# yeyupiaoling/MASR

Measured on AMD Instinct MI355X. Metric: audio-seconds/sec (RTF^-1), conformer_streaming_fbank b32x10s, PCM->fbank->encoder->ctc_greedy->text, higher is better.
Workload: dtype f32; 1 GPU; configs[1]: conformer.yml streaming fbank, batch=32 synthetic 16 kHz 10 s utterances per GPU, ctc_greedy, random-init weights V=4233; global_batch=32, parallelism=dp1, world_size_observed=1, backend=none

## Files before the change

include/masr_hip.h:

```cpp
#ifndef MASR_HIP_H
#define MASR_HIP_H
#include <stdint.h>
#ifdef __cplusplus
extern "C" {
#endif

typedef struct masr_engine masr_engine;

typedef struct masr_config {
    int32_t model_kind;
    int32_t d_model;
    int32_t heads;
    int32_t d_ff;
    int32_t num_blocks;
    int32_t cnn_kernel;
    int32_t n_mels;
    int32_t vocab_size;
    int32_t causal;
    int32_t max_pos;
    int32_t device_id;
    int32_t reserved[5];
} masr_config;

const char* masr_last_error(void);
// ... 121 lines not shown

int masr_stream_open(masr_engine* e, int32_t max_frames_out, int32_t* stream_id);
int masr_stream_reset(masr_engine* e, int32_t stream_id);
int masr_stream_close(masr_engine* e, int32_t stream_id);
int masr_stream_set_history(masr_engine* e, int32_t stream_id, int32_t required_cache_size);
int masr_stream_offset(masr_engine* e, int32_t stream_id, int32_t* offset);
int masr_stream_cache_len(masr_engine* e, int32_t stream_id, int32_t* cache_len);
int masr_stream_room(masr_engine* e, int32_t stream_id, int32_t* frames_left);

int masr_stage_rows(void* dst, int64_t row_bytes, const void* const* src, const int32_t* n_samples, int32_t B, int32_t sample_bytes,
                    int32_t threads);

int masr_resample_f32(const float* x, int64_t n_orig, double ratio, const double* win, const double* dwin, int64_t nwin,
                      int32_t num_table, float* y, int64_t n_out);
int masr_resample_rows(masr_engine* e, const void* src_dev, int32_t sample_format, int64_t src_stride, const int32_t* rows_host,
                       const int32_t* rows_dev, int32_t R, double ratio, const double* table_dev, int64_t nwin, int32_t num_table,
                       float* dst_dev, int32_t dst_rows, int64_t dst_stride, void* stream);
int masr_encode_chunk(masr_engine* e, const int32_t* stream_ids, int32_t n, const float* feats_dev, int32_t Tc,
                      float* probs_dev, int32_t* argmax_dev, float* maxprob_dev, void* stream);
int masr_stream_export_cache(masr_engine* e, int32_t stream_id, float* att_dev, float* cnn_dev, void* stream);

int masr_op_layernorm(masr_engine* e, const float* x_dev, const float* w_dev, const float* b_dev, float* y_dev,
                      int32_t M, float eps, void* stream);
int masr_op_gemm(masr_engine* e, const float* a_dev, const float* w_dev, const float* bias_dev, const float* res_dev,
                 float* c_dev, int32_t M, int32_t N, int32_t K, int32_t act, float alpha, void* stream);

#define MASR_SIDE_STREAMS 5
int masr_side_stream(masr_engine* e, int32_t kind, void** stream_out);

#define MASR_LANES 2
int masr_select_lane(masr_engine* e, int32_t lane);

int masr_debug_set(masr_engine* e, int32_t key, int32_t value);

int masr_profile_select(masr_engine* e, int32_t kind);
int masr_profile_read(masr_engine* e, double* total_ms, int64_t* launches, double* flops, int32_t reset);

int masr_mfma_order_probe(const float* a_dev, const float* b_dev, float* c32_dev, float* c16_dev, int32_t k, const int32_t* perm,
                          void* stream);

#ifdef __cplusplus
}
#endif
#endif
```

masr_amd/_lib.py:

```python
import ctypes as C
import os

from .build import LIB_PATH

_lib = None


class MasrConfig(C.Structure):
    _fields_ = [('model_kind', C.c_int32), ('d_model', C.c_int32), ('heads', C.c_int32), ('d_ff', C.c_int32),
                ('num_blocks', C.c_int32), ('cnn_kernel', C.c_int32), ('n_mels', C.c_int32),
                ('vocab_size', C.c_int32), ('causal', C.c_int32), ('max_pos', C.c_int32), ('device_id', C.c_int32),
                ('reserved', C.c_int32 * 5)]


class MasrError(RuntimeError):
    pass


_P = C.c_void_p
_I = C.c_int32
_F = C.c_float

SIGNATURES = {
    'masr_last_error': [],
# ... 43 lines not shown
    'masr_vad_forward': [_P, _I, _P, _I, _I, _I, _P, _P, _P, _P],
    'masr_mean_square': [_P, _P, _I, _P, _I, _I, _P, _P],
    'masr_mfcc_batch': [_P, _P, _I, _P, _I, _I, _I, _F, _I, _P, _P, _P, _P],
    'masr_linear_batch': [_P, _P, _I, _P, _I, _I, _I, _F, _P, _P, _P, _P],
    'masr_transcribe_batch': [_P, _P, _P, _I, _I, _I, _F, _I, _P, _P, _P, _P],
    'masr_transcribe_rows': [_P, _P, _I, _P, _I, _I, _I, _F, _P, _I, _P, _P],
    'masr_pool_create': [_P, _I, _I, _I, _F, _I, C.POINTER(_P)],
    'masr_pool_destroy': [_P],
    'masr_pool_open': [_P, C.POINTER(_I)],
    'masr_pool_close': [_P, _I],
    'masr_pool_reset': [_P, _I],
    'masr_pool_step': [_P, _I, _P, _P, _P, _P, _P, _P, _P, C.POINTER(_I), C.POINTER(_P), C.POINTER(_P), C.POINTER(_P),
                       C.POINTER(_I), C.POINTER(_P), _P],
    'masr_pool_profile': [_P, C.POINTER(C.c_double), C.POINTER(C.c_int64), _I],
    'masr_encoder_frames': [_P, _I, C.POINTER(_I)],
    'masr_engine_info': [_P, C.POINTER(_I), C.POINTER(_I), C.POINTER(_I)],
    'masr_stream_open': [_P, _I, C.POINTER(_I)],
    'masr_stream_reset': [_P, _I],
    'masr_stream_close': [_P, _I],
    'masr_stream_offset': [_P, _I, C.POINTER(_I)],
    'masr_stream_cache_len': [_P, _I, C.POINTER(_I)],
    'masr_stream_room': [_P, _I, C.POINTER(_I)],
    'masr_resample_f32': [_P, C.c_int64, C.c_double, _P, _P, C.c_int64, _I, _P, C.c_int64],
    'masr_resample_rows': [_P, _P, _I, C.c_int64, _P, _P, _I, C.c_double, _P, C.c_int64, _I, _P, _I, C.c_int64, _P],
    'masr_stream_set_history': [_P, _I, _I],
    'masr_encode_chunk': [_P, C.POINTER(_I), _I, _P, _I, _P, _P, _P, _P],
    'masr_stream_export_cache': [_P, _I, _P, _P, _P],
    'masr_op_layernorm': [_P, _P, _P, _P, _P, _I, _F, _P],
    'masr_op_gemm': [_P, _P, _P, _P, _P, _P, _I, _I, _I, _I, _F, _P],
    'masr_side_stream': [_P, _I, C.POINTER(_P)],
    'masr_select_lane': [_P, _I],
    'masr_stage_rows': [_P, C.c_int64, _P, _P, _I, _I, _I],
    'masr_debug_set': [_P, _I, _I],
    'masr_mfma_order_probe': [_P, _P, _P, _P, _I, _P, _P],
    'masr_profile_select': [_P, _I],
    'masr_profile_read': [_P, C.POINTER(C.c_double), C.POINTER(C.c_int64), C.POINTER(C.c_double), _I],
}
_RESTYPE = {'masr_last_error': C.c_char_p, 'masr_destroy': None, 'masr_beam_destroy': None, 'masr_lm_destroy': None,
            'masr_lm_last_error': C.c_char_p, 'masr_vad_last_error': C.c_char_p, 'masr_vad_destroy': None, 'masr_pool_destroy': None}


GAIN_FN = C.CFUNCTYPE(C.c_int, C.POINTER(C.c_float), C.c_int32, C.c_float, C.POINTER(C.c_float), C.c_void_p)


def lib():
    global _lib
    if _lib is not None:
        return _lib
    import torch
    if not os.path.exists(LIB_PATH):
        raise MasrError(f'{LIB_PATH} not found: build it with `python -m masr_amd.build` '
                        f'(hipcc --offload-arch=gfx950). There is no CPU fallback.')
    h = C.CDLL(LIB_PATH)
    for name, args in SIGNATURES.items():
        fn = getattr(h, name)
        fn.argtypes = args
        fn.restype = _RESTYPE.get(name, C.c_int)
    _lib = h
    return h


def check(rc):
    if rc != 0:
        raise MasrError(lib().masr_last_error().decode('utf-8', 'replace'))
```

masr_amd/build.py:

```python
import os
import subprocess
from concurrent.futures import ThreadPoolExecutor

ROOT = os.path.dirname(os.path.abspath(__file__))
CSRC = os.path.join(ROOT, 'csrc')
LIB_DIR = os.path.join(ROOT, 'lib')
LIB_PATH = os.path.join(LIB_DIR, 'libmasr_hip.so')
SOURCES = ['gemm_f32.hip', 'ffn_reduce.hip', 'ffn_pc.hip', 'sqz_layer.hip', 'rowgemm.hip', 'rowgemm_small.hip', 'elementwise.hip',
           'attention.hip', 'lstm.hip', 'gru.hip', 'beam_gpu.hip', 'lm_scorer.cpp', 'fbank.hip', 'silero.hip', 'engine.hip', 'pool.hip',
           'beam_search.cpp', 'stage.cpp', 'resample.cpp', 'resample.hip']
EXPERIMENTS = os.environ.get('MASR_BUILD_EXPERIMENTS') == '1'
EXPERIMENT_SOURCES = ['gemm_bf16x3.hip', 'ffn_x3.hip', 'ffn_coop.hip', 'ffn_dual.hip']
if EXPERIMENTS:
    SOURCES = SOURCES + EXPERIMENT_SOURCES
HEADERS = [os.path.join(CSRC, 'common.h'), os.path.join(CSRC, 'lm_scorer.h'),
           os.path.join(os.path.dirname(ROOT), 'include', 'masr_hip.h')]
FLAGS = ['--offload-arch=gfx950', '-O3', '-std=c++17', '-fPIC', '-Wno-unused-value'] + (['-DMASR_EXPERIMENTS=1'] if EXPERIMENTS else [])
FILE_FLAGS = {'resample.hip': ['-ffp-contract=off', '-fno-gpu-flush-denormals-to-zero']}
STAMP = os.path.join(LIB_DIR, '.build_flavour')


def _hipcc():
    for c in (os.environ.get('HIPCC'), '/opt/rocm/bin/hipcc', 'hipcc'):
        if c and (os.path.isabs(c) and os.path.exists(c) or not os.path.isabs(c)):
            return c
    return 'hipcc'


def _sources():
    return [s for s in SOURCES if os.path.exists(os.path.join(CSRC, s))]


def _obj(src):
    stem, ext = os.path.splitext(src)
    if sum(os.path.splitext(s)[0] == stem for s in SOURCES) > 1:
        stem += '_' + ext[1:]
    return os.path.join(LIB_DIR, stem + '.o')


def _stale(src):
    obj = _obj(src)
# ... 60 lines not shown
```

masr_amd/csrc/common.h:

```cpp
#pragma once
#include <hip/hip_runtime.h>
#include <stdint.h>

#include "lm_scorer.h"

#ifndef MASR_EXPERIMENTS
#define MASR_EXPERIMENTS 0
#endif

typedef float f32x4 __attribute__((ext_vector_type(4)));
typedef float f32x16 __attribute__((ext_vector_type(16)));

namespace masr {

struct LdsAttr {
    size_t granted[32] = {};
};
void ensure_dynamic_lds(const void* fn, size_t bytes, LdsAttr& st);
void note_launch_error(const char* what, hipError_t e);

#ifdef __HIPCC__
struct SeqRow {
    int b, t;
};
__device__ __forceinline__ SeqRow seq_row(int b0, int t0, int T, int lr) {
    SeqRow r{b0, t0 + lr};
    while (r.t >= T) {
        r.t -= T;
        ++r.b;
    }
    return r;
}

__device__ __forceinline__ float wave_sum_dpp(float v) {
#define MASR_DPP_F(x, ctrl, rows) \
    __builtin_bit_cast(float, __builtin_amdgcn_update_dpp(0, __builtin_bit_cast(int, (x)), (ctrl), (rows), 0xf, false))
    v += MASR_DPP_F(v, 0x111, 0xf);
    v += MASR_DPP_F(v, 0x112, 0xf);
    v += MASR_DPP_F(v, 0x114, 0xf);
    v += MASR_DPP_F(v, 0x118, 0xf);
    v += MASR_DPP_F(v, 0x142, 0xa);
    v += MASR_DPP_F(v, 0x143, 0xc);
#undef MASR_DPP_F
    return __builtin_bit_cast(float, __builtin_amdgcn_readlane(__builtin_bit_cast(int, v), 63));
}
#endif


enum InputLayer { IL_CONV2D = 0, IL_CONV2D6 = 1, IL_CONV2D8 = 2 };
__host__ __device__ inline int sub_rate(int il) { return il == IL_CONV2D6 ? 6 : il == IL_CONV2D8 ? 8 : 4; }
__host__ __device__ inline int sub_min_frames(int il) { return il == IL_CONV2D6 ? 11 : il == IL_CONV2D8 ? 15 : 7; }
__host__ __device__ inline int sub_after_conv1(int il, int n1) {
    return il == IL_CONV2D6 ? (n1 - 2) / 3 : il == IL_CONV2D8 ? ((n1 - 1) / 2 - 1) / 2 : (n1 - 1) / 2;
}
__host__ __device__ inline int sub_frames(int il, int T) { return T < sub_min_frames(il) ? 0 : sub_after_conv1(il, (T - 1) / 2); }
__host__ __device__ inline int sub_bins(int il, int F) { return sub_after_conv1(il, (F - 1) / 2); }

enum GemmAct { ACT_NONE = 0, ACT_RELU = 1, ACT_SILU = 2 };
enum GemmAMode { A_PLAIN = 0, A_CONV2 = 1, A_CONV5 = 2 };
enum GemmEpi { EPI_STD = 0, EPI_GLU = 1, EPI_SPLITK = 2 };

struct GemmArgs {
    const float* A;
    const float* W;
    const float* bias;
    float* C;
    const float* R;
    const int* lens;
    int M, N, K;
    int lda, ldc, ldr;
    int act;
    float alpha;
    int mask_tp;
    int bias_after_alpha;
    int T1, F1, T2, F2, Cc;
    int nsplit, ksplit;
    int skip_rps, skip_div;
    const float* Wp;
// ... 123 lines not shown
    const float* lnb;
    const float* W;
    const float* bias;
    float* out;
    int N, ldo;
    const float* pre_lnw;
    const float* pre_lnb;
    long plane_stride;
    int seq_t, pad_t;
};
struct FfnHead {
    const float* glu;
    const float* dw_w;
    const float* dw_b;
    const float* lnw;
    const float* lnb;
    const float* gconst;
    const float* W;
    const float* bias;
    const int* lens;
    int seq_t, ktaps, mstride;
    float* xout;
};
int launch_ffn_fused(float* x, const float* lnw, const float* lnb, const float* w1, const float* b1, const float* w2,
                     const float* b2, int M, int dff, float eps, float scale, int affine_prologue, float* partial,
                     int nsplit, hipStream_t s, const FfnPostLn* post = nullptr, const FfnTail* tail = nullptr,
                     const FfnHead* head = nullptr, bool packed = false);
void launch_pack_ffn_pc(const float* w1, const float* w2, float* p1, float* p2, int dff, hipStream_t s);
void launch_pack_rows_pc(const float* w, float* p, int N, hipStream_t s, int n_src = -1);
int launch_ffn16(float* x, const float* lnw, const float* lnb, const float* w1, const float* b1, const float* w2, const float* b2, int M,
                 int dff, float eps, float scale, hipStream_t s, const FfnTail* tail, const FfnHead* head);
void launch_pack_ffn16(const float* w1, const float* w2, float* p1, float* p2, int dff, hipStream_t s);
void launch_pack_rows16(const float* w, float* p, int N, hipStream_t s, int n_src = -1);
struct SqzStageArgs {
    float* x;
    float* out;
    const float* att;
    const float* head_w;
    const float* head_b;
    const float *ln_a_w, *ln_a_b, *ln_b_w, *ln_b_b;
    const float *ffn_s, *ffn_b, *w1, *b1, *w2, *b2;
    const float *tail_w, *tail_b, *tail_s, *tail_sb;
    float* tail_out;
    float* glu_out;
    const float* glu;
    const float *dw_w, *dw_b, *bn_scale, *bn_shift, *gconst;
    const float* gpad;
    const int* lens;
    int M, dff, seq_t, mstride, ktaps, tail_n, glu_pad_l, glu_pad_tot;
    float eps;
    int skip_pad;
};
bool launch_sqz_stage(const SqzStageArgs& a, int stage, hipStream_t s);
#if MASR_EXPERIMENTS
int launch_ffn_dual(float* x, const float* lnw, const float* lnb, const float* p1, const float* b1, const float* p2,
                    const float* b2, int M, int dff, float eps, float scale, int affine_prologue, hipStream_t s,
                    const FfnTail* tail, const FfnHead* head);
void launch_pack_ffn_dual(const float* w1, const float* w2, float* p1, float* p2, int dff, hipStream_t s);
void launch_pack_rows_dual(const float* w, float* p, hipStream_t s);
#else
inline int launch_ffn_dual(float*, const float*, const float*, const float*, const float*, const float*, const float*, int, int, float,
                           float, int, hipStream_t, const FfnTail*, const FfnHead*) { return -1; }
inline void launch_pack_ffn_dual(const float*, const float*, float*, float*, int, hipStream_t) {}
inline void launch_pack_rows_dual(const float*, float*, hipStream_t) {}
#endif

// ... 129 lines not shown
```

masr_amd/csrc/engine.hip:

```cpp
#include <math.h>
#include <stdio.h>
#include <stdlib.h>
#include <string.h>

#include <map>
#include <mutex>
#include <string>
#include <vector>

#include "../../include/masr_hip.h"
#include "common.h"

using namespace masr;
namespace masr {
int lm_device_view(masr_lm* lm, LmView* out);
bool lm_word_based(const masr_lm* lm);
}
extern "C" const char* masr_lm_last_error(void);

static thread_local std::string g_err;
static int fail(const std::string& m) {
    g_err = m;
    return 1;
}
// ... 199 lines not shown
static int clear_sync(void* p, int value, size_t n) {
    HIPCHK(hipMemset(p, value, n));
    HIPCHK(hipStreamSynchronize(nullptr));
    return 0;
}

struct masr_engine : EngineWs {
    masr_config cfg;
    EngineWs parked[MASR_LANES];
    int lane = 0;
    hipEvent_t pack_ev = nullptr;
    void* pack_stream = nullptr;
    bool pack_pending = false;
    bool finalized = false;
    std::map<std::string, HostTensor> host;
    std::vector<void*> owned;
    float *cmvn_mean = nullptr, *cmvn_istd = nullptr, *conv1_w = nullptr, *conv1_b = nullptr, *conv2_w = nullptr,
          *conv2_b = nullptr, *conv3_w = nullptr, *conv3_b = nullptr, *embed_w = nullptr, *embed_b = nullptr, *after_w = nullptr, *after_b = nullptr,
          *ctc_w = nullptr, *ctc_b = nullptr, *pe = nullptr;
    std::vector<LayerW> layers;
    std::vector<SqLayerW> sq_layers;
    std::vector<Ds2LayerW> ds2_layers;
    std::vector<GBeam> gbeams;
    DevBuf beam_pool, beam_state;
    std::map<void*, std::pair<DevBuf, DevBuf>> beam_ws;
    std::map<void*, DevBuf> ms_ws;
    int skip_padding = 7;
    void* beam_first_stream = nullptr;
    bool beam_first_set = false;
    std::map<const float*, std::pair<DevBuf, DevBuf>> ffn_packed;
    std::map<const float*, std::pair<DevBuf, DevBuf>> ffn_dual_packed;
    std::map<const float*, std::pair<DevBuf, DevBuf>> x3_packed;
    std::map<const float*, std::pair<DevBuf, DevBuf>> ffn16_packed;
    std::map<const float*, std::pair<DevBuf, DevBuf>> conv2_packed;
    long long* beam_prof = nullptr;
    float *preln_w = nullptr, *preln_b = nullptr, *tr_dw_w = nullptr, *tr_dw_b = nullptr, *tr_pw_w = nullptr,
          *tr_pw_b = nullptr, *rec_w = nullptr, *rec_b = nullptr;
    int reduce_idx = -1, recover_idx = -1;
    int stride_idx = -1, n_group_layers = 0, group_size = 3;
    int input_layer = IL_CONV2D;
    bool conv_bn = false;
    bool ds2_gru = false;
    float *window = nullptr, *melwt = nullptr, *tw512 = nullptr, *twr4 = nullptr;
    FbankTables fbank_tables() const { return FbankTables{window, melwt, tw512, twr4, mel_lo}; }
    int* mel_lo = nullptr;
    float *dct = nullptr, *lifter = nullptr;
    int dct_ceps = 0;
    double *lin_win = nullptr, *lin_tw = nullptr;
    double lin_scale = 0.0;
    std::vector<Stream> streams;
    int prof_kind = 0;
    int prof_stride = 1, prof_seen = 0;
    std::vector<std::pair<hipEvent_t, hipEvent_t>> prof_events;
    size_t prof_used = 0;
    double prof_flops = 0.0;
};

namespace {

template <class T>
int upload(masr_engine* e, const std::vector<T>& v, T** out) {
    void* p = nullptr;
    HIPCHK(hipMalloc(&p, std::max<size_t>(v.size(), 1) * sizeof(T)));
    HIPCHK(hipMemcpy(p, v.data(), v.size() * sizeof(T), hipMemcpyHostToDevice));
    e->owned.push_back(p);
    *out = reinterpret_cast<T*>(p);
// ... 59 lines not shown
        }
    }
    ~CallGuard() {
        if (packed_count(e) == n0) return;
        if (!e->pack_ev && hipEventCreateWithFlags(&e->pack_ev, hipEventDisableTiming) != hipSuccess) return;
        if (hipEventRecord(e->pack_ev, s) == hipSuccess) {
            e->pack_stream = (void*)s;
            e->pack_pending = true;
        }
    }
};

static int g_ffn_dual = 0;
static int g_ffn_packed = 2;
static int g_ffn16 = 1;
static int g_conv2_rows = 1;
static int g_conv1_fused = 1;
static int g_embed_rows = 1;
static int g_bf16x3 = 0;

void gemm(masr_engine* e, hipStream_t s, const float* A, int lda, const float* W, const float* bias, float* C, int ldc,
          int M, int N, int K, int act, float alpha, const float* R, int ldr, int kind = PROF_GEMM,
          const int* lens = nullptr, int mask_tp = 0) {
    GemmArgs a{};
    a.A = A; a.W = W; a.bias = bias; a.C = C; a.R = R; a.lens = lens;
    a.M = M; a.N = N; a.K = K; a.lda = lda; a.ldc = ldc; a.ldr = ldr;
    a.act = act; a.alpha = alpha; a.mask_tp = mask_tp;
    ProfScope ps(e, s, kind, 2.0 * M * (double)N * K);
    if (g_bf16x3 && launch_gemm_bf16x3(a, A_PLAIN, s)) return;
    launch_gemm(a, A_PLAIN, EPI_STD, s);
}

static int g_rowgemm_packed = 1;
const float* packed_rows_of(masr_engine* e, const float* W, int N, hipStream_t s) {
    auto it = e->ffn_packed.find(W);
    if (it == e->ffn_packed.end()) {
        const int Np = (N + 255) / 256 * 256;
        std::pair<DevBuf, DevBuf> pk;
        if (pk.first.ensure((size_t)Np * 256 * sizeof(float))) return nullptr;
        launch_pack_rows_pc(W, pk.first.as<float>(), Np, s, N);
        it = e->ffn_packed.emplace(W, pk).first;
    }
    return it->second.first.as<float>();
}

int packed_ffn_of(masr_engine* e, const float* w1, const float* w2, hipStream_t s, const float** p1, const float** p2) {
    const int d = e->cfg.d_model;
    auto it = e->ffn_packed.find(w1);
    if (it == e->ffn_packed.end()) {
        std::pair<DevBuf, DevBuf> pk;
        CHK(pk.first.ensure((size_t)e->cfg.d_ff * d * sizeof(float)));
        CHK(pk.second.ensure((size_t)e->cfg.d_ff * d * sizeof(float)));
        launch_pack_ffn_pc(w1, w2, pk.first.as<float>(), pk.second.as<float>(), e->cfg.d_ff, s);
        it = e->ffn_packed.emplace(w1, pk).first;
    }
    *p1 = it->second.first.as<float>();
    *p2 = it->second.second.as<float>();
    return 0;
}
static bool sqz_stage_supported(const masr_engine* e) {
    const int K = e->cfg.cnn_kernel;
    return e->cfg.d_model == 256 && e->cfg.d_ff % 128 == 0 && e->cfg.d_ff >= 256 && (K == 31 || K == 15);
}

void rowgemm(masr_engine* e, hipStream_t s, int pro, int epi, const float* A, int lda, const float* lnw,
             const float* lnb, const float* W, const float* bias, float* C, int ldc, int M, int N, const float* R,
// ... 852 lines not shown
            launch_rowgemm(a, RG_PRO_PLAIN, RG_EPI_GLU, s);
        }
    }
    if (pw2_later) return 0;
    {
        RowGemmArgs a{};
        a.A = e->glu.as<float>(); a.lda = d; a.lnw = w.cln_w; a.lnb = w.cln_b; a.dw_w = w.dw_w; a.dw_b = w.dw_b;
        a.W = w.pw2_w; a.bias = w.pw2_b; a.C = x; a.ldc = d; a.R = x; a.ldr = d; a.M = M; a.N = d; a.alpha = 1.f;
        a.eps = 1e-5f; a.mstride = 4; a.seq_t = Tq; a.pad = pad;
        ProfScope ps(e, s, PROF_GEMM, 2.0 * M * (double)d * d);
        if (!launch_rowgemm(a, RG_PRO_DWCONV, RG_EPI_RESID, s)) {
            launch_dwconv_ln_silu(e->glu.as<float>(), w.dw_w, w.dw_b, w.cln_w, w.cln_b, e->dwo.as<float>(), n, Tq, K, 1e-5f, s,
                                  nullptr);
            a.A = e->dwo.as<float>();
            launch_rowgemm(a, RG_PRO_PLAIN, RG_EPI_RESID, s);
        }
    }
    return 0;
}

void mhsa(masr_engine* e, hipStream_t s, const LayerW& w, int M, const AttSeq* kv_seqs = nullptr, int kv_tq = 0) {
    const int d = e->cfg.d_model;
    rowgemm(e, s, RG_PRO_LN, RG_EPI_STORE, e->x.as<float>(), d, w.ln_mha_w, w.ln_mha_b, w.wqkv, w.bqkv, e->qkv.as<float>(),
            3 * d, M, 3 * d, nullptr, 0, 1.f, nullptr, 0, 0, 0, nullptr, nullptr, PROF_GEMM, 4, 0, 0, 0, 0, 0, 0, 0, kv_seqs, kv_tq);
}
void mhsa_out(masr_engine* e, hipStream_t s, const LayerW& w, int M) {
    const int d = e->cfg.d_model;
    float* x = e->x.as<float>();
    rowgemm(e, s, RG_PRO_PLAIN, RG_EPI_RESID, e->att.as<float>(), d, nullptr, nullptr, w.wo, w.bo, x, d, M, d, x, d, 1.f,
            nullptr, 0, 0, 0, nullptr, nullptr);
}

void mhsa_out_pw1(masr_engine* e, hipStream_t s, const LayerW& w, const EncodeCtx& c, int mstride = 4, int K = 0,
                  const float* att = nullptr, int a_seq_t = 0, int a_seq_stride = 0) {
    const int d = e->cfg.d_model, pad = (K > 0 ? K : e->cfg.cnn_kernel) - 1, M = c.nseq * c.Tq;
    float* x = e->x.as<float>();
    RowGemmArgs a{};
    a.A = att ? att : e->att.as<float>(); a.lda = d; a.a_seq_t = a_seq_t; a.a_seq_stride = a_seq_stride; a.lnw = w.ln_conv_w; a.lnb = w.ln_conv_b; a.W = w.chain_w; a.bias = w.chain_b;
    a.C = e->glu.as<float>(); a.ldc = d; a.M = M; a.N = 3 * d; a.R = x; a.R2 = x; a.ldr = d; a.alpha = 1.f;
    a.lens = c.lens; a.seq_t = c.Tq; a.mstride = mstride; a.eps = 1e-5f;
    a.out_seq_t = c.Tq; a.out_pad_l = e->cfg.causal ? pad : pad / 2; a.out_pad_tot = pad;
    if (g_rowgemm_packed) a.Wp = packed_rows_of(e, w.chain_w, 3 * d, s);
    ProfScope ps(e, s, PROF_GEMM, 2.0 * M * (double)(3 * d) * d);
    launch_rowgemm(a, RG_PRO_PLAIN, RG_EPI_CHAIN, s);
}

}

static int upload_conv_frontend(masr_engine* e, const std::string& c1, const std::string& c2, const std::string& proj) {
    const int d = e->cfg.d_model, F = e->cfg.n_mels, F1 = (F - 1) / 2, F2 = (F1 - 1) / 2;
    const HostTensor* t;
    CHK(up(e, "encoder.global_cmvn.mean", {F}, &e->cmvn_mean));
    CHK(up(e, "encoder.global_cmvn.istd", {F}, &e->cmvn_istd));
    CHK(get(e, c1 + ".weight", {d, 1, 3, 3}, &t));
    {
        std::vector<float> w(9 * d);
        for (int c = 0; c < d; ++c)
            for (int k = 0; k < 9; ++k) w[k * d + c] = t->v[c * 9 + k];
        CHK(upload(e, w, &e->conv1_w));
    }
    CHK(up(e, c1 + ".bias", {d}, &e->conv1_b));
    CHK(get(e, c2 + ".weight", {d, d, 3, 3}, &t));
    {
        std::vector<float> w((size_t)d * 9 * d);
        for (int co = 0; co < d; ++co)
            for (int ci = 0; ci < d; ++ci)
                for (int k = 0; k < 9; ++k)
                    w[(size_t)co * 9 * d + (size_t)(ci / 32) * 9 * 32 + k * 32 + ci % 32] = t->v[((size_t)co * d + ci) * 9 + k];
        CHK(upload(e, w, &e->conv2_w));
    }
    CHK(up(e, c2 + ".bias", {d}, &e->conv2_b));
    CHK(get(e, proj + ".weight", {d, (int64_t)d * F2}, &t));
    {
        std::vector<float> w((size_t)d * d * F2);
        for (int o = 0; o < d; ++o)
            for (int c = 0; c < d; ++c)
// ... 529 lines not shown
                &qkv_done));
        if (!qkv_done) mhsa(e, s, w, M);
        const bool fuse_ac = g_attn_chain && !few_rows && !g_no_chain && !e->conv_bn && H == 4 && d == 256 && g_rowgemm_packed;
        if (fuse_ac) {
            AttnChainArgs a{};
            a.seqs = e->attseq.as<AttSeq>(); a.nseq = B; a.q_stride = 3 * d; a.kv_stride = 3 * d;
            a.chunk_size = (decoding_chunk_size > 0 && e->cfg.causal) ? decoding_chunk_size : 0; a.pos_stride = 1;
            a.ptab = w.ptab; a.bias_u = w.pos_u; a.bias_v = w.pos_v;
            a.Wp = packed_rows_of(e, w.chain_w, 3 * d, s); a.bias = w.chain_b; a.lnw = w.ln_conv_w; a.lnb = w.ln_conv_b;
            a.R = x; a.R2 = x; a.C = e->glu.as<float>(); a.lens = feat_lens_dev; a.seq_t = Tq; a.mstride = 4;
            a.out_pad_l = e->cfg.causal ? pad : pad / 2; a.out_pad_tot = pad; a.eps = 1e-5f;
            if (!a.Wp) return fail("packed chain weights: allocation failed");
            ProfScope ps(e, s, PROF_ATT, 6.0 * d * (double)Tq * Tq * B + 2.0 * M * (double)(3 * d) * d);
            launch_attn_chain(a, Tq, s);
        } else {
            ProfScope ps(e, s, PROF_ATT, 6.0 * d * (double)Tq * Tq * B);
            launch_attention(e->attseq.as<AttSeq>(), B, Tq, H, 3 * d, 3 * d, w.ptab, w.pos_u, w.pos_v,
                             (decoding_chunk_size > 0 && e->cfg.causal) ? decoding_chunk_size : 0, 1, s);
        }
        if (few_rows) {
            mhsa_out(e, s, w, M);
            const bool fuse = g_split_head && e->cfg.cnn_kernel == 15 && g_ffn_packed >= 2 && !g_no_ffn_head && !e->conv_bn;
            CHK(conv_module(e, s, w, ctx, false, 0, 4, false, fuse));
            const FfnHead head{e->glu.as<float>(), w.dw_w, w.dw_b, w.cln_w, w.cln_b, e->cfg.causal ? w.gconst : nullptr,
                               w.pw2_w, w.pw2_b, feat_lens_dev, Tq, e->cfg.cnn_kernel, 4, nullptr};
            CHK(ffn(e, s, M, w.ln_ff_w, w.ln_ff_b, w.ff_w1, w.ff_b1, w.ff_w2, w.ff_b2, 0.5f, 0, w.ln_fin_w, w.ln_fin_b, x, nullptr,
                    nullptr, fuse ? &head : nullptr));
            continue;
        } else if (g_no_chain || e->conv_bn) {
            mhsa_out(e, s, w, M);
            CHK(conv_module(e, s, w, ctx, false));
            CHK(ffn(e, s, M, w.ln_ff_w, w.ln_ff_b, w.ff_w1, w.ff_b1, w.ff_w2, w.ff_b2));
        } else {
            if (!fuse_ac) mhsa_out_pw1(e, s, w, ctx);
            const FfnHead head{e->glu.as<float>(), w.dw_w, w.dw_b, w.cln_w, w.cln_b, e->cfg.causal ? w.gconst : nullptr,
                               w.pw2_w, w.pw2_b, feat_lens_dev, Tq, e->cfg.cnn_kernel, 4, nullptr};
            CHK(ffn(e, s, M, w.ln_ff_w, w.ln_ff_b, w.ff_w1, w.ff_b1, w.ff_w2, w.ff_b2, 0.5f, 0, nullptr, nullptr, nullptr, nullptr,
                    nullptr, &head));
        }
        prev = &w;
    }
    if (prev) launch_layernorm(x, prev->ln_fin_w, prev->ln_fin_b, x, M, 1e-5f, 0, 0, nullptr, s);
    launch_layernorm(x, e->after_w, e->after_b, enc_out_dev, M, 1e-5f, 0, 0, nullptr, s);
    LAUNCHCHK();
    return 0;
}

static int g_ctc_fused_blocks = 160;
static int ctc_head(masr_engine* e, const float* enc_dev, int M, float* probs_dev, int write_probs, int32_t* argmax_dev,
                    float* maxprob_dev, hipStream_t s) {
    const int d = enc_dim(e), V = e->cfg.vocab_size;
    float* logits = probs_dev;
    if (!logits) {
        CHK(e->logits.ensure((size_t)M * V * sizeof(float)));
        logits = e->logits.as<float>();
    }
    gemm(e, s, enc_dev, d, e->ctc_w, e->ctc_b, logits, V, M, V, d, ACT_NONE, 1.f, nullptr, 0);
    launch_softmax_argmax(logits, M, V, V, write_probs, argmax_dev, maxprob_dev, s);
    LAUNCHCHK();
    return 0;
}

int masr_ctc_probs(masr_engine* e, const float* enc_dev, int32_t M, float* probs_dev, int32_t* argmax_dev,
                   float* maxprob_dev, void* stream) {
    if (!e || !e->finalized) return fail("engine not finalized");
    ENTER(e);
    CallGuard call_guard(e, (hipStream_t)stream);
// ... 1018 lines not shown
        return fail("masr_debug_set: this key selects an experimental kernel that is not in this build (MASR_BUILD_EXPERIMENTS=1)");
#endif
    if (key == 1) set_ffn_variant(value);
    else if (key == 5) g_no_chain = value;
    else if (key == 6) set_rowgemm_small(value);
    else if (key == 7) set_attention_fewq(value);
    else if (key == 14) set_attention_fold(value);
    else if (key == 15) g_embed_split = value;
    else if (key == 19) g_hot_weights = value;
    else if (key == 20) g_bf16x3 = value;
    else if (key == 21) set_gemm_bf16x3_waves(value);
    else if (key == 22) set_ffn_x3_rotation(value);
    else if (key == 23) g_ffn_packed = value;
    else if (key == 24) g_ffn_dual = value;
    else if (key == 25) g_rowgemm_packed = value;
    else if (key == 26) set_attention_grouped_fold(value);
    else if (key == 27) g_ctc_fused_blocks = value;
    else if (key == 28) set_attention_fewq_wgs(value);
    else if (key == 29) g_few_rows_path = value;
    else if (key == 30) g_split_head = value;
    else if (key == 31) g_efficient_fused = value;
    else if (key == 32) g_beam_lm_cache = value;
    else if (key == 33) set_conv2_mid_fill(value);
    else if (key == 34) g_attn_chain = value;
    else if (key == 35) g_ffn_coop = value;
    else if (key == 36) g_sqz_fused_blocks = value;
    else if (key == 37) g_beam_narrow = value;
    else if (key == 38) e->skip_padding = value;
    else if (key == 39) g_ffn16 = value;
    else if (key == 40) g_conv2_rows = value;
    else if (key == 41) g_conv1_fused = value;
    else if (key == 42) g_embed_rows = value;
    else if (key == 43) set_gru_mfma_units(value);
    else if (key == 17) set_gemm_waves(value);
    else if (key == 18) set_conv1_nt(value);
    else if (key == 16) { e->prof_stride = value > 1 ? value : 1; e->prof_seen = 0; }
    else if (key == 8) g_no_ffn_tail = value;
    else if (key == 9) g_no_ffn_head = value;
    else if (key == 12) set_rowgemm_small_blocks(value);
    else if (key == 13) g_ffn_split_blocks = value;
    else if (key == 2) {
        if (value) {
            if (!e->beam_prof) {
                void* p = nullptr;
                HIPCHK(hipMalloc(&p, 16 * sizeof(long long)));
                e->owned.push_back(p);
                e->beam_prof = (long long*)p;
            }
        } else if (e->beam_prof) {
            long long h[16];
            HIPCHK(hipMemcpy(h, e->beam_prof, sizeof(h), hipMemcpyDeviceToHost));
            fprintf(stderr, "beam phases (cycles, last workgroup): setup+hash %lld  extensions %lld  prefixes+count %lld  select %lld  compact %lld\n",
                    h[0], h[1], h[2], h[3], h[4]);
            fprintf(stderr, "  narrow step (%lld frames): tables+candidates %lld  hash+contexts %lld  children+scorer table %lld  extensions %lld  "
                    "prefixes+select %lld  scan %lld  survivors %lld  new prefixes %lld\n", h[5], h[6], h[7], h[8], h[9], h[10], h[11], h[12], h[13]);
            if (h[15] > 0) fprintf(stderr, "  wide step (%lld frames): %.1f distinct scorer contexts per frame\n", h[15], (double)h[14] / (double)h[15]);
            e->beam_prof = nullptr;
        }
    }
    else return fail("unknown debug key");
    return 0;
}

int masr_profile_select(masr_engine* e, int32_t kind) {
    if (!e) return fail("null engine");
    e->prof_kind = kind;
    return 0;
}

int masr_profile_read(masr_engine* e, double* total_ms, int64_t* launches, double* flops, int32_t reset) {
    if (!e) return fail("null engine");
    ENTER(e);
    double tot = 0.0;
    for (size_t i = 0; i < e->prof_used; ++i) {
        HIPCHK(hipEventSynchronize(e->prof_events[i].second));
        float ms = 0.f;
        HIPCHK(hipEventElapsedTime(&ms, e->prof_events[i].first, e->prof_events[i].second));
        tot += ms;
    }
    if (total_ms) *total_ms = tot;
    if (launches) *launches = (int64_t)e->prof_used;
    if (flops) *flops = e->prof_flops;
    if (reset) {
        e->prof_used = 0;
        e->prof_flops = 0.0;
    }
    return 0;
}

}
```

masr_amd/csrc/ffn_pc.hip:

```cpp
#include "common.h"

namespace masr {

static constexpr int PC_BM = 32;
static constexpr int PC_D = 256;
static constexpr int PC_CH = 128;
static constexpr int PC_XLD = PC_D + 4;
static constexpr int PC_HLD = PC_CH + 4;
static constexpr int PC_WLD = 32 + 4;
static constexpr int PC_WSLAB = 32 * PC_WLD;
static constexpr int PC_NSET = 4;
#ifdef PC_NOFENCE_PACKED
#define PC_FENCE(var) do { if ((var) != 2) __builtin_amdgcn_sched_barrier(0); } while (0)
#else
#define PC_FENCE(var) __builtin_amdgcn_sched_barrier(0)
#endif

#ifndef PC_BUFLOAD
#define PC_BUFLOAD 1
#endif
__device__ __forceinline__ f32x4 pc_bufld(__amdgpu_buffer_rsrc_t rs, unsigned lane16, unsigned float_index) {
    return __builtin_bit_cast(f32x4, __builtin_amdgcn_raw_buffer_load_b128(rs, lane16, float_index * 4u, 0));
}

// ... 486 lines not shown
                            if ((slot & 3) == 3) pre[j % PC_NSET][g] = tld(t + (j + PC_NSET) / 8, (j + PC_NSET) & 7, g);
                        } else if (slot < 8) {
                            if ((slot & 1) == 0) *reinterpret_cast<f32x4*>(dst_of(j + 1, slot >> 1)) = pre[pset][slot >> 1];
                        } else if ((slot & 1) == 0) {
                            pre[pset][(slot - 8) >> 1] = *reinterpret_cast<const f32x4*>(
                                tsrc(t + (j + 1 + PC_NSET) / 8, (j + 1 + PC_NSET) & 7, (slot - 8) >> 1));
                        }
                        __builtin_amdgcn_sched_barrier(0);
                    }
                }
            }
            if (col < tail.N && tail.plane_stride > 0) {
                float* plane = tail.out + (size_t)t * tail.plane_stride + wave * 32 + frow;
                const int pb0 = row0 / tail.seq_t, pt0 = row0 - pb0 * tail.seq_t;
#pragma unroll
                for (int r = 0; r < 16; ++r) {
                    const int lr = (r & 3) + 8 * (r >> 2) + 4 * fh;
                    const SeqRow q = seq_row(pb0, pt0, tail.seq_t, lr);
                    if (row0 + lr < M) plane[((size_t)q.b * (tail.seq_t + tail.pad_t) + q.t) * 256] = acc[r] + bv;
                }
            } else if (col < tail.N) {
#pragma unroll
                for (int r = 0; r < 16; ++r) {
                    const int row = row0 + (r & 3) + 8 * (r >> 2) + 4 * fh;
                    if (row < M) tail.out[(size_t)row * tail.ldo + col] = acc[r] + bv;
                }
            }
        }
    }
}


static constexpr int P16_BM = 16;
static constexpr int P16_RING = 8;
__host__ __device__ constexpr int p16_k0(int kk) { return (kk & 1) * 4 + (kk >> 1); }

template <int TAIL, int HEADK>
__global__ __launch_bounds__(512) __attribute__((amdgpu_waves_per_eu(4))) void ffn16_kernel(
    float* x, const float* __restrict__ lnw, const float* __restrict__ lnb, const float* __restrict__ w1, const float* __restrict__ b1,
    const float* __restrict__ w2, const float* __restrict__ b2, int M, int dff, float eps, float scale, FfnTail tail, FfnHead head) {
    extern __shared__ __align__(16) float sm[];
    float* xn = sm;
    float* hs = xn + P16_BM * PC_XLD;

    const int tid = threadIdx.x, lane = tid & 63;
    const int wave = __builtin_amdgcn_readfirstlane(tid >> 6);
    const int role = wave >> 2, idx = wave & 3;
    const int row0 = blockIdx.x * P16_BM;
    const int fr = lane & 15, kk = lane >> 4, ko = p16_k0(kk);
    const unsigned lane16 = lane * 16;
    f32x4 pre[P16_RING];
    const float* xa = xn + fr * PC_XLD + ko;

    f32x4 gw_head = {0.f, 0.f, 0.f, 0.f}, gb_head = gw_head;
    if (HEADK > 0) {
        {
            constexpr int KT = HEADK > 0 ? HEADK : 1, pad = KT - 1;
            const int c = tid & 255, half = tid >> 8;
            float w[KT], win[KT], nw[8];
#pragma unroll
            for (int j = 0; j < KT; ++j) w[j] = head.dw_w[j * 256 + c];
            const float bv = head.dw_b[c];
            const float gc = head.gconst ? head.gconst[c] : 0.f;
            const bool has_gc = head.gconst != nullptr;
            const int hb0 = row0 / head.seq_t, ht0 = row0 - hb0 * head.seq_t, lr_last = M - 1 - row0;
#pragma unroll
            for (int rr = 0; rr < 8; ++rr) {
                const SeqRow q = seq_row(hb0, ht0, head.seq_t, min(half * 8 + rr, lr_last));
// ... 512 lines not shown
```

Measured before the change: 52730 audio-seconds/sec.

## Add 16-row MFMA kernel for attention-out projection chained with LN and pointwise conv1 GLU

Adds a new rowgemm16 kernel that does the MHSA output projection plus residual, the conv-module layernorm, and the pointwise-conv1 GLU in one block of 16 rows. It uses MFMA 16x16x4 f32 with a register ring of prefetched packed weights, in the same style as the ffn16 kernel. The intent is more blocks in flight and better weight streaming than the generic packed rowgemm chain when M is large. The weights are repacked into the 16-row layout once and cached, and the old path is kept as a fallback with a debug toggle and a launch counter.

```diff
diff --git a/include/masr_hip.h b/include/masr_hip.h
--- a/include/masr_hip.h
+++ b/include/masr_hip.h
@@ -177,6 +177,7 @@
 int masr_select_lane(masr_engine* e, int32_t lane);
 
 int masr_debug_set(masr_engine* e, int32_t key, int32_t value);
+int masr_debug_get(masr_engine* e, int32_t key, int64_t* value);
 
 int masr_profile_select(masr_engine* e, int32_t kind);
 int masr_profile_read(masr_engine* e, double* total_ms, int64_t* launches, double* flops, int32_t reset);
diff --git a/masr_amd/_lib.py b/masr_amd/_lib.py
--- a/masr_amd/_lib.py
+++ b/masr_amd/_lib.py
@@ -99,6 +99,7 @@
     'masr_select_lane': [_P, _I],
     'masr_stage_rows': [_P, C.c_int64, _P, _P, _I, _I, _I],
     'masr_debug_set': [_P, _I, _I],
+    'masr_debug_get': [_P, _I, C.POINTER(C.c_int64)],
     'masr_mfma_order_probe': [_P, _P, _P, _P, _I, _P, _P],
     'masr_profile_select': [_P, _I],
     'masr_profile_read': [_P, C.POINTER(C.c_double), C.POINTER(C.c_int64), C.POINTER(C.c_double), _I],
diff --git a/masr_amd/build.py b/masr_amd/build.py
--- a/masr_amd/build.py
+++ b/masr_amd/build.py
@@ -6,7 +6,7 @@
 CSRC = os.path.join(ROOT, 'csrc')
 LIB_DIR = os.path.join(ROOT, 'lib')
 LIB_PATH = os.path.join(LIB_DIR, 'libmasr_hip.so')
-SOURCES = ['gemm_f32.hip', 'ffn_reduce.hip', 'ffn_pc.hip', 'sqz_layer.hip', 'rowgemm.hip', 'rowgemm_small.hip', 'elementwise.hip',
+SOURCES = ['gemm_f32.hip', 'ffn_reduce.hip', 'ffn_pc.hip', 'sqz_layer.hip', 'rowgemm.hip', 'rowgemm16.hip', 'rowgemm_small.hip', 'elementwise.hip',
            'attention.hip', 'lstm.hip', 'gru.hip', 'beam_gpu.hip', 'lm_scorer.cpp', 'fbank.hip', 'silero.hip', 'engine.hip', 'pool.hip',
            'beam_search.cpp', 'stage.cpp', 'resample.cpp', 'resample.hip']
 EXPERIMENTS = os.environ.get('MASR_BUILD_EXPERIMENTS') == '1'
diff --git a/masr_amd/csrc/common.h b/masr_amd/csrc/common.h
--- a/masr_amd/csrc/common.h
+++ b/masr_amd/csrc/common.h
@@ -44,6 +44,8 @@
 #undef MASR_DPP_F
     return __builtin_bit_cast(float, __builtin_amdgcn_readlane(__builtin_bit_cast(int, v), 63));
 }
+static constexpr int P16_RING = 8;
+__host__ __device__ constexpr int p16_k0(int kk) { return (kk & 1) * 4 + (kk >> 1); }
 #endif
 
 
@@ -233,6 +235,7 @@
                  int dff, float eps, float scale, hipStream_t s, const FfnTail* tail, const FfnHead* head);
 void launch_pack_ffn16(const float* w1, const float* w2, float* p1, float* p2, int dff, hipStream_t s);
 void launch_pack_rows16(const float* w, float* p, int N, hipStream_t s, int n_src = -1);
+bool launch_rowgemm16_chain(const RowGemmArgs& a, hipStream_t s);
 struct SqzStageArgs {
     float* x;
     float* out;
diff --git a/masr_amd/csrc/engine.hip b/masr_amd/csrc/engine.hip
--- a/masr_amd/csrc/engine.hip
+++ b/masr_amd/csrc/engine.hip
@@ -255,6 +255,7 @@
     std::map<const float*, std::pair<DevBuf, DevBuf>> ffn_dual_packed;
     std::map<const float*, std::pair<DevBuf, DevBuf>> x3_packed;
     std::map<const float*, std::pair<DevBuf, DevBuf>> ffn16_packed;
+    long long rowgemm16_launches = 0;
     std::map<const float*, std::pair<DevBuf, DevBuf>> conv2_packed;
     long long* beam_prof = nullptr;
     float *preln_w = nullptr, *preln_b = nullptr, *tr_dw_w = nullptr, *tr_dw_b = nullptr, *tr_pw_w = nullptr,
@@ -380,6 +381,7 @@
 }
 
 static int g_rowgemm_packed = 1;
+static int g_rowgemm16 = 1;
 const float* packed_rows_of(masr_engine* e, const float* W, int N, hipStream_t s) {
     auto it = e->ffn_packed.find(W);
     if (it == e->ffn_packed.end()) {
@@ -1298,7 +1300,7 @@
 }
 
 void mhsa_out_pw1(masr_engine* e, hipStream_t s, const LayerW& w, const EncodeCtx& c, int mstride = 4, int K = 0,
-                  const float* att = nullptr, int a_seq_t = 0, int a_seq_stride = 0) {
+                  const float* att = nullptr, int a_seq_t = 0, int a_seq_stride = 0, bool rows16 = false) {
     const int d = e->cfg.d_model, pad = (K > 0 ? K : e->cfg.cnn_kernel) - 1, M = c.nseq * c.Tq;
     float* x = e->x.as<float>();
     RowGemmArgs a{};
@@ -1306,8 +1308,26 @@
     a.C = e->glu.as<float>(); a.ldc = d; a.M = M; a.N = 3 * d; a.R = x; a.R2 = x; a.ldr = d; a.alpha = 1.f;
     a.lens = c.lens; a.seq_t = c.Tq; a.mstride = mstride; a.eps = 1e-5f;
     a.out_seq_t = c.Tq; a.out_pad_l = e->cfg.causal ? pad : pad / 2; a.out_pad_tot = pad;
+    ProfScope ps(e, s, PROF_GEMM, 2.0 * M * (double)(3 * d) * d);
+    if (rows16 && g_rowgemm16 && g_rowgemm_packed && d == 256 && M >= 112 * 32 && a_seq_t == 0) {
+        auto it = e->ffn16_packed.find(w.chain_w);
+        if (it == e->ffn16_packed.end()) {
+            std::pair<DevBuf, DevBuf> pk;
+            if (!pk.first.ensure((size_t)3 * d * d * sizeof(float))) {
+                launch_pack_rows16(w.chain_w, pk.first.as<float>(), 3 * d, s);
+                it = e->ffn16_packed.emplace(w.chain_w, pk).first;
+            }
+        }
+        if (it != e->ffn16_packed.end()) {
+            a.Wp = it->second.first.as<float>();
+            if (launch_rowgemm16_chain(a, s)) {
+                e->rowgemm16_launches++;
+                return;
+            }
+            a.Wp = nullptr;
+        }
+    }
     if (g_rowgemm_packed) a.Wp = packed_rows_of(e, w.chain_w, 3 * d, s);
-    ProfScope ps(e, s, PROF_GEMM, 2.0 * M * (double)(3 * d) * d);
     launch_rowgemm(a, RG_PRO_PLAIN, RG_EPI_CHAIN, s);
 }
 
@@ -1903,7 +1923,7 @@
             CHK(conv_module(e, s, w, ctx, false));
             CHK(ffn(e, s, M, w.ln_ff_w, w.ln_ff_b, w.ff_w1, w.ff_b1, w.ff_w2, w.ff_b2));
         } else {
-            if (!fuse_ac) mhsa_out_pw1(e, s, w, ctx);
+            if (!fuse_ac) mhsa_out_pw1(e, s, w, ctx, 4, 0, nullptr, 0, 0, true);
             const FfnHead head{e->glu.as<float>(), w.dw_w, w.dw_b, w.cln_w, w.cln_b, e->cfg.causal ? w.gconst : nullptr,
                                w.pw2_w, w.pw2_b, feat_lens_dev, Tq, e->cfg.cnn_kernel, 4, nullptr};
             CHK(ffn(e, s, M, w.ln_ff_w, w.ln_ff_b, w.ff_w1, w.ff_b1, w.ff_w2, w.ff_b2, 0.5f, 0, nullptr, nullptr, nullptr, nullptr,
@@ -2988,6 +3008,7 @@
     else if (key == 41) g_conv1_fused = value;
     else if (key == 42) g_embed_rows = value;
     else if (key == 43) set_gru_mfma_units(value);
+    else if (key == 44) g_rowgemm16 = value;
     else if (key == 17) set_gemm_waves(value);
     else if (key == 18) set_conv1_nt(value);
     else if (key == 16) { e->prof_stride = value > 1 ? value : 1; e->prof_seen = 0; }
@@ -3018,6 +3039,13 @@
     return 0;
 }
 
+int masr_debug_get(masr_engine* e, int32_t key, int64_t* value) {
+    if (!e || !value) return fail("null argument");
+    if (key == 44) *value = e->rowgemm16_launches;
+    else return fail("masr_debug_get: unknown key");
+    return 0;
+}
+
 int masr_profile_select(masr_engine* e, int32_t kind) {
     if (!e) return fail("null engine");
     e->prof_kind = kind;
diff --git a/masr_amd/csrc/ffn_pc.hip b/masr_amd/csrc/ffn_pc.hip
--- a/masr_amd/csrc/ffn_pc.hip
+++ b/masr_amd/csrc/ffn_pc.hip
@@ -542,8 +542,6 @@
 
 
 static constexpr int P16_BM = 16;
-static constexpr int P16_RING = 8;
-__host__ __device__ constexpr int p16_k0(int kk) { return (kk & 1) * 4 + (kk >> 1); }
 
 template <int TAIL, int HEADK>
 __global__ __launch_bounds__(512) __attribute__((amdgpu_waves_per_eu(4))) void ffn16_kernel(
diff --git a/masr_amd/csrc/rowgemm16.hip b/masr_amd/csrc/rowgemm16.hip
--- /dev/null
+++ b/masr_amd/csrc/rowgemm16.hip
@@ -0,0 +1,157 @@
+#include "common.h"
+
+namespace masr {
+
+static constexpr int R16_BM = 16;
+static constexpr int R16_K = 256;
+static constexpr int R16_LD = R16_K + 4;
+
+__global__ __launch_bounds__(512) __attribute__((amdgpu_waves_per_eu(4))) void rowgemm16_chain_kernel(RowGemmArgs p) {
+    extern __shared__ __align__(16) float sm[];
+    float* at = sm;
+    float* xt = at + R16_BM * R16_LD;
+
+    const int tid = threadIdx.x, lane = tid & 63;
+    const int wave = __builtin_amdgcn_readfirstlane(tid >> 6);
+    const int row0 = blockIdx.x * R16_BM;
+    const int fr = lane & 15, kk = lane >> 4, ko = p16_k0(kk);
+    const unsigned lane16 = lane * 16;
+
+    f32x4 v2[2];
+#pragma unroll
+    for (int rr = 0; rr < 2; ++rr) {
+        const int row = row0 + wave * 2 + rr;
+        v2[rr] = *reinterpret_cast<const f32x4*>(p.A + (size_t)(row < p.M ? row : 0) * p.lda + lane * 4);
+    }
+    const __amdgpu_buffer_rsrc_t wrs = __builtin_amdgcn_make_buffer_rsrc(const_cast<float*>(p.Wp), 0, 3 * 256 * R16_K * 4, 0x00020000);
+    auto wld = [&](int t, int f) -> f32x4 {
+        const unsigned fi = (unsigned)((min(t, 2) * 8 + wave) * 32 + f) * 256u;
+        return __builtin_bit_cast(f32x4, __builtin_amdgcn_raw_buffer_load_b128(wrs, lane16, fi * 4u, 0));
+    };
+    f32x4 pre[P16_RING];
+#pragma unroll
+    for (int k = 0; k < P16_RING; ++k) pre[k] = wld(0, k);
+    const f32x4 gw = *reinterpret_cast<const f32x4*>(p.lnw + lane * 4);
+    const f32x4 gb = *reinterpret_cast<const f32x4*>(p.lnb + lane * 4);
+    float bo[2], ba[2], bg[2], res0[8];
+#pragma unroll
+    for (int nt = 0; nt < 2; ++nt) {
+        const int ch = wave * 32 + 16 * nt + fr;
+        bo[nt] = p.bias[ch];
+        ba[nt] = p.bias[256 + ch];
+        bg[nt] = p.bias[512 + ch];
+#pragma unroll
+        for (int r = 0; r < 4; ++r) {
+            const int row = min(row0 + 4 * kk + r, p.M - 1);
+            res0[4 * nt + r] = p.R[(size_t)row * p.ldr + ch];
+        }
+    }
+    bool live2[2];
+    {
+        const int cb0 = p.seq_t > 0 ? row0 / p.seq_t : 0, ct0 = p.seq_t > 0 ? row0 - cb0 * p.seq_t : 0;
+#pragma unroll
+        for (int rr = 0; rr < 2; ++rr) {
+            const int lr = wave * 2 + rr;
+            bool live = row0 + lr < p.M;
+            if (live && p.lens && p.seq_t > 0) {
+                const SeqRow q = seq_row(cb0, ct0, p.seq_t, lr);
+                live = p.mstride * q.t < p.lens[q.b];
+            }
+            live2[rr] = live;
+        }
+    }
+#pragma unroll
+    for (int rr = 0; rr < 2; ++rr) {
+        const int lr = wave * 2 + rr;
+        *reinterpret_cast<f32x4*>(&at[lr * R16_LD + lane * 4]) = row0 + lr < p.M ? v2[rr] : f32x4{0.f, 0.f, 0.f, 0.f};
+    }
+    __syncthreads();
+
+    auto tile = [&](int t, const float* xa, f32x4 (&acc)[2]) {
+        acc[0] = f32x4{0.f, 0.f, 0.f, 0.f};
+        acc[1] = f32x4{0.f, 0.f, 0.f, 0.f};
+        float a0 = xa[0], a1 = xa[2];
+#pragma unroll
+        for (int g = 0; g < 32; ++g) {
+            float n0 = 0.f, n1 = 0.f;
+            if (g + 1 < 32) { n0 = xa[8 * (g + 1)]; n1 = xa[8 * (g + 1) + 2]; }
+#pragma unroll
+            for (int q = 0; q < 4; ++q) {
+                acc[q & 1] = __builtin_amdgcn_mfma_f32_16x16x4f32(q < 2 ? a0 : a1, pre[g % P16_RING][q], acc[q & 1], 0, 0, 0);
+                if (q == 3 && (t < 2 || g + P16_RING < 32)) pre[g % P16_RING] = wld(t + (g + P16_RING) / 32, (g + P16_RING) & 31);
+                __builtin_amdgcn_sched_barrier(0);
+            }
+            a0 = n0;
+            a1 = n1;
+        }
+    };
+
+    f32x4 acc[2], accv[2];
+    tile(0, at + fr * R16_LD + ko, acc);
+#pragma unroll
+    for (int nt = 0; nt < 2; ++nt) {
+        const int ch = wave * 32 + 16 * nt + fr;
+#pragma unroll
+        for (int r = 0; r < 4; ++r) {
+            const int lr = 4 * kk + r;
+            const float v = res0[4 * nt + r] + (acc[nt][r] + bo[nt]);
+            if (row0 + lr < p.M) p.R2[(size_t)(row0 + lr) * p.ldr + ch] = v;
+            xt[lr * R16_LD + ch] = v;
+        }
+    }
+    __syncthreads();
+#pragma unroll
+    for (int rr = 0; rr < 2; ++rr) {
+        const int lr = wave * 2 + rr;
+        const f32x4 v = *reinterpret_cast<const f32x4*>(&xt[lr * R16_LD + lane * 4]);
+        const float mean = wave_sum_dpp(v[0] + v[1] + v[2] + v[3]) * (1.0f / 256.0f);
+        const float d0 = v[0] - mean, d1 = v[1] - mean, d2 = v[2] - mean, d3 = v[3] - mean;
+        const float var = wave_sum_dpp(d0 * d0 + d1 * d1 + d2 * d2 + d3 * d3) * (1.0f / 256.0f);
+        const float rstd = 1.0f / sqrtf(var + p.eps);
+        f32x4 o;
+        o[0] = d0 * rstd * gw[0] + gb[0];
+        o[1] = d1 * rstd * gw[1] + gb[1];
+        o[2] = d2 * rstd * gw[2] + gb[2];
+        o[3] = d3 * rstd * gw[3] + gb[3];
+        if (!live2[rr]) o = f32x4{0.f, 0.f, 0.f, 0.f};
+        *reinterpret_cast<f32x4*>(&xt[lr * R16_LD + lane * 4]) = o;
+    }
+    __syncthreads();
+
+    const float* xa = xt + fr * R16_LD + ko;
+    tile(1, xa, accv);
+    tile(2, xa, acc);
+    size_t crow[4];
+    {
+        const int ob0 = p.out_seq_t > 0 ? row0 / p.out_seq_t : 0, ot0 = p.out_seq_t > 0 ? row0 - ob0 * p.out_seq_t : 0;
+#pragma unroll
+        for (int r = 0; r < 4; ++r) {
+            const int lr = 4 * kk + r;
+            crow[r] = row0 + lr;
+            if (p.out_seq_t > 0) {
+                const SeqRow q = seq_row(ob0, ot0, p.out_seq_t, lr);
+                crow[r] = (size_t)q.b * (p.out_seq_t + p.out_pad_tot) + p.out_pad_l + q.t;
+            }
+        }
+    }
+#pragma unroll
+    for (int nt = 0; nt < 2; ++nt) {
+        const int ch = wave * 32 + 16 * nt + fr;
+#pragma unroll
+        for (int r = 0; r < 4; ++r) {
+            if (row0 + 4 * kk + r >= p.M) continue;
+            const float g = acc[nt][r] + bg[nt];
+            p.C[crow[r] * p.ldc + ch] = (accv[nt][r] + ba[nt]) * __builtin_amdgcn_rcpf(1.0f + __expf(-g));
+        }
+    }
+}
+
+bool launch_rowgemm16_chain(const RowGemmArgs& a, hipStream_t s) {
+    if (a.M <= 0) return true;
+    if (!a.Wp || a.N != 3 * R16_K || a.a_seq_t > 0 || !a.lnw || !a.lnb || !a.bias || !a.R || !a.R2) return false;
+    const size_t lds = (size_t)2 * R16_BM * R16_LD * sizeof(float);
+    hipLaunchKernelGGL(rowgemm16_chain_kernel, dim3((a.M + R16_BM - 1) / R16_BM), dim3(512), lds, s, a);
+    return true;
+}
+
+}
```

After: 52970 audio-seconds/sec, median of 6. About the same (+0.5%).
